# michaelfeil/skyjo_rl

Hardware: AMD Instinct MI355X
Metric: env-steps/sec (whole node) at 65 536 parallel 3-player games (higher is better)
Workload: dtype int8

## Files before the change

### skyjo_rl_amd/csrc/skyjo_step.h

```cpp
#pragma once
#ifndef SKYJO_DEVICE_PARTS
#error "include skyjo_device.h"
#endif

__device__ __forceinline__ void sk_publish_deals(const SkParams &P, int g) {
  const size_t G = (size_t)P.tiles * SK_TILE;
  const int b = P.busy[g];
  if (b) {
    const uint32_t tag = P.plan_tag[g];
    const uint32_t f = __hip_atomic_load(&P.done_flag[g], __ATOMIC_RELAXED, __HIP_MEMORY_SCOPE_AGENT);
    if ((f & 0x7fffffffu) == tag) {
      SK_FENCE_ACQUIRE(P);
      if (!P.cancel[g] && f == tag) P.spare_ready[(size_t)(b - 1) * G + g] = 1;
      P.busy[g] = 0, P.cancel[g] = 0;
    }
  }
}
__device__ __forceinline__ void sk_plan_deals(const SkParams &P, int g, int lane) {
  const size_t G = (size_t)P.tiles * SK_TILE;
  bool need = false, empty = false;
  if (g < P.B) {
    const uint8_t busy = P.busy[g];
    const int head = P.bank_head[g] % SK_BANK;
    const uint32_t consumed = P.deals_consumed[g];
    uint8_t ready[SK_BANK];
#pragma unroll
    for (int k = 0; k < SK_BANK; k++) ready[k] = P.spare_ready[(size_t)k * G + g];
    bool open = true;
    int r = 0;
#pragma unroll
    for (int k = 0; k < SK_BANK; k++) {
      uint8_t f = 0;
#pragma unroll
      for (int j = 0; j < SK_BANK; j++) f = (head + k) % SK_BANK == j ? ready[j] : f;
      open = open && f != 0;
      r += open ? 1 : 0;
    }
    need = !busy && r < SK_BANK;
    empty = need && r == 0;
    if (need) {
      P.busy[g] = (uint8_t)(1 + (head + r) % SK_BANK);
      P.cancel[g] = 0;
      P.plan_ep[g] = consumed + (uint32_t)r;
      P.plan_tag[g] = P.plan_new_tag;
    }
  }
  const unsigned long long be = __ballot(empty);
  if (be && lane == 0) atomicAdd(P.bank_empty + (P.be_add & 1u), (uint32_t)__popcll(be));
}

__device__ __forceinline__ void sk_error_to_host(const SkParams &P, int lane) {
  if (lane == 0) {
    const uint32_t e = __hip_atomic_load(P.dev_error, __ATOMIC_RELAXED, __HIP_MEMORY_SCOPE_AGENT);
    if (e) P.health_host[2] = e;
  }
}
__device__ __forceinline__ void sk_export_raw(const SkParams &P, uint8_t *lp, int g, uint8_t *o) {
  for (int c = 0; c < P.L.chunks; c++) ((uint4 *)o)[c] = LQ(c);
  double *d = (double *)(o + P.L.state_bytes);
  for (int p = 0; p < P.L.N; p++) d[p] = P.rewards[(size_t)g * P.L.N + p], d[P.L.N + p] = P.scores[(size_t)g * P.L.N + p];
  uint32_t *m = (uint32_t *)(d + 2 * P.L.N);
  m[0] = P.rng_mode == SKYJO_RNG_MT19937 ? (uint32_t)P.mt_idx[g] : 0u;
  m[1] = P.done[g];
}

__device__ __forceinline__ uint32_t sk_next_tag(uint32_t t) {
  t = (t + 1u) & 0x7fffffffu;
  return t ? t : 1u;
}
template <bool INDIRECT, bool POLICY, int NP, bool PLANAR = false>
__device__ __forceinline__ void step_body(const SkParams &Pin, const int tile, const int lane, uint32_t *lds_raw, const int32_t *actions,
                                          uint8_t *rec_out, int32_t *act_out, int iters, uint64_t policy_seed, uint64_t iter0,
                                          double *end_rew_out, uint8_t *end_out, uint8_t *raw_out, int raw_stride, const int cycle_len = 0,
                                          const bool defer_ok = true) {
  SkParams P = Pin;
  TRACE_DECL;
  if (NP > 0) P.L = sk_make_layout(NP, INDIRECT ? 1 : 0);
  const int g = tile * SK_TILE + lane;
  const uint32_t lds_tile = (uint32_t)(uintptr_t)(__attribute__((address_space(3))) uint32_t *)lds_raw;
  uint8_t *lp = (uint8_t *)lds_raw + lane * 16;
  uint8_t *stg = (uint8_t *)lds_raw + P.L.chunks * 1024;
  uint8_t *fp = stg + lane * 4;
  const int stg_bytes = (INDIRECT || PLANAR) ? 4096 : SK_TILE * (P.L.rec_bytes + 16);
  uint8_t *ap = stg + stg_bytes + lane * 8;
  constexpr bool DEFER = POLICY && NP > 0 && NP < 8;
  constexpr bool REGACC = NP > 0 && NP < 8;
  constexpr int NACC = REGACC ? SK_ACC_KINDS * NP : 1;
  double racc_store[NACC];
#pragma unroll
  for (int k = 0; k < NACC; k++) racc_store[k] = 0.0;
  double *racc = REGACC ? racc_store : nullptr;
  uint8_t *pendp = DEFER && defer_ok ? stg + stg_bytes + (REGACC ? 0 : SK_ACC_KINDS * P.L.N * 512) + lane * 16 : nullptr;
  int pend_fin = -1;
  if (!REGACC)
    for (int k = 0; k < SK_ACC_KINDS * P.L.N; k++) ACC(k) = 0.0;
  STAMP_DECL;
  if (!POLICY) tile_load(P, P.state, tile, lane, lp);
  else dma_record<true>((const uint8_t *)P.state, (uint32_t)((((size_t)tile * P.L.chunks) * SK_TILE + lane) * 16), lds_tile, P.L.chunks);
  if (P.ov_flags & 1u) sk_publish_deals(P, g);
  sk_vm_drain();
  HdrRegs h;
  HDR_LOAD(h);
  STAMP(0);
  const bool valid = ((h.w0 >> 16) & F_VALID) != 0;
  LaneCounters cnt;
  uint32_t r0 = 0, r1 = 0, r2 = 0, r3 = 0;
  const uint64_t gid = P.game_id0 + (uint64_t)g;
  ObsRegs ob;
  if (valid) obs_load(P, lp, (h.w0 >> 8) & 0xff, ob);
  for (int it = 0; it < iters; it++) {
    const uint64_t iter = iter0 + (uint64_t)it;
    if (POLICY && (it == 0 || (iter & 3) == 0)) {
      philox4x32_10((uint32_t)(iter >> 2), (uint32_t)gid, (uint32_t)(gid >> 32), 0x504F4C00u, (uint32_t)policy_seed,
                    (uint32_t)(policy_seed >> 32), r0, r1, r2, r3);
      for (int k = (int)(iter & 3); k > 0; k--) {
        const uint32_t t = r0;
        r0 = r1, r1 = r2, r2 = r3, r3 = t;
      }
    }
    STAMP_T(3);
    const uint32_t word = r0;
    if (POLICY) {
      r0 = r1, r1 = r2, r2 = r3, r3 = word;
    }
    int a = -1;
    if (valid) {
      const bool over = ((h.w0 >> 16) & F_DONE) != 0;
      if (!POLICY) a = actions[g];
      const bool skip = !POLICY && a == SKYJO_ACTION_SKIP;
      const bool acted = !over && !skip;
      SpareRegs sp;
      const bool resetting = over && P.auto_reset && !skip;
      if (resetting) spare_issue(P, lp, lds_tile, tile, lane, g, sp);
      STAMP_T(4);
      if (!over && !skip) {
        const uint32_t v0 = ob.q0, v1 = ob.q1, v2 = ob.q2;
        STAMP_N(2);
        const uint4 row_pre = LQ(sk_pb(P.L, (h.w0 >> 8) & 0xff) >> 4);
        asm volatile("" ::: "memory");
        if (POLICY) a = policy_pick(h.w0 & 0xff, ob, word);
#ifndef SK_STAMPS_FINE
        STAMP_N(3);
#endif
        apply_action<INDIRECT, NP, POLICY>(P, lp, fp, ap, h, v0, v1, v2, a, g, cnt, st, pendp, pend_fin, row_pre, racc);
#ifdef SK_STAMPS_FINE
        STAMP(6);
#else
        STAMP(5);
#endif
      } else if (!skip) {
        a = -1;
        if (P.auto_reset) {
          bool dealt = true;
          if (!spare_commit(P, lp, g, sp)) {
            dealt = deal_inline(P, lp, fp, g, tile, lane, sp.head);
            cnt.waits++;
          }
          HDR_LOAD(h);
          if (SK_OFTEN(dealt)) {
            h.w0 = (h.w0 & 0x00ffffffu) | ((uint32_t)SKYJO_ST_RESET << 24);
            cnt.resets++;
          }
        } else {
          h.w0 = (h.w0 & 0x00ffffffu) | ((uint32_t)SKYJO_ST_NOOP_DONE << 24);
        }
        STAMP(1);
      } else {
        a = -1;
      }
      if (!POLICY && acted && (unsigned)a >= (unsigned)SKYJO_NUM_ACTIONS) a = -2;
      if (!POLICY && end_out) {
        const bool end = acted && ((h.w0 >> 16) & F_DONE) != 0;
        end_out[g] = end ? 1 : 0;
        for (int q = 0; q < P.L.N; q++) end_rew_out[(size_t)g * P.L.N + q] = end ? P.rewards[(size_t)g * P.L.N + q] : 0.0;
      }
      const uint4 rec_a = LQ(1);
      const uint32_t rec_b = LB(32);
      const uint4 rec_row = LQ((sk_pb(P.L, (h.w0 >> 8) & 0xff) + PB_VIS) >> 4);
      asm volatile("" ::: "memory");
      obs_from_row(rec_row, ob);
      if (rec_out) {
        if (INDIRECT) {
          uint4 rr[4];
          emit_record<INDIRECT>(P, lp, h, ob, a, nullptr, rr, &rec_a, rec_b);
          if (PLANAR) {
            typedef uint32_t u32x4_t __attribute__((ext_vector_type(4)));
            uint8_t *blk = rec_out + ((size_t)it * P.tiles + (size_t)tile) * (SK_TILE * 64) + lane * 16;
#pragma unroll
            for (int p = 0; p < 4; p++) __builtin_nontemporal_store((u32x4_t){rr[p].x, rr[p].y, rr[p].z, rr[p].w}, (u32x4_t *)(blk + p * 1024));
          } else {
#pragma unroll
            for (int p = 0; p < 4; p++) *(uint4 *)(stg + lane * 64 + ((p + (lane >> 1)) & 3) * 16) = rr[p];
          }
        } else if (PLANAR) {
          constexpr int PIECES = NP > 0 ? (((19 + 12 * NP + 3) & ~3) + 32 + 15) / 16 : 1;
          uint32_t wbuf[4 * PIECES];
#pragma unroll
          for (int k = 0; k < 4 * PIECES; k++) wbuf[k] = 0u;
          emit_record<INDIRECT>(P, lp, h, ob, a, (uint8_t *)wbuf, nullptr, &rec_a, rec_b);
          typedef uint32_t u32x4_t __attribute__((ext_vector_type(4)));
          uint8_t *blk = rec_out + ((size_t)it * P.tiles + (size_t)tile) * (SK_TILE * 16 * PIECES) + lane * 16;
#pragma unroll
          for (int p = 0; p < PIECES; p++)
            __builtin_nontemporal_store((u32x4_t){wbuf[4 * p], wbuf[4 * p + 1], wbuf[4 * p + 2], wbuf[4 * p + 3]}, (u32x4_t *)(blk + p * 1024));
        } else {
          emit_record<INDIRECT>(P, lp, h, ob, a, stg + lane * sk_stage_stride(P.L.rec_bytes), nullptr, &rec_a, rec_b);
        }
      }
      if (act_out) __builtin_nontemporal_store(a, &act_out[(size_t)it * P.B + g]);
#ifdef SK_STAMPS_FINE
      STAMP(7);
#else
      STAMP(6);
#endif
    }
    if (DEFER && ((it & (SK_SCORE_EVERY - 1)) == SK_SCORE_EVERY - 1 || it == iters - 1)) {
      if (SK_RARE(__any(pend_fin >= 0))) {
        if (pend_fin >= 0) {
          finish_game_fixed<(NP > 0 && NP < 8) ? NP : 1>(P, pendp, 1024, ap, g, pend_fin, racc);
          pend_fin = -1;
        }
      }
    }
    if (!INDIRECT && !PLANAR && rec_out) {
      typedef uint32_t u32x4_t __attribute__((ext_vector_type(4)));
      const int pieces = P.L.rec_bytes >> 4, stride = sk_stage_stride(P.L.rec_bytes);
      uint8_t *blk = rec_out + ((size_t)it * P.B + (size_t)tile * SK_TILE) * (size_t)P.L.rec_bytes;
      const int live = P.B - tile * SK_TILE;
      for (int q0 = lane; q0 < pieces * SK_TILE; q0 += 4 * SK_TILE) {
        uint4 v[4];
#pragma unroll
        for (int j = 0; j < 4; j++) {
          const int q = q0 + j * SK_TILE, r = q / pieces, p = q - r * pieces;
          if (q < pieces * SK_TILE) v[j] = *(const uint4 *)(stg + r * stride + p * 16);
        }
        if (SK_OFTEN(live >= SK_TILE)) {
#pragma unroll
          for (int j = 0; j < 4; j++) {
            const int q = q0 + j * SK_TILE;
            if (q0 - lane + j * SK_TILE < pieces * SK_TILE)
              __builtin_nontemporal_store((u32x4_t){v[j].x, v[j].y, v[j].z, v[j].w}, (u32x4_t *)(blk + (size_t)q * 16));
          }
        } else {
#pragma unroll
          for (int j = 0; j < 4; j++) {
            const int q = q0 + j * SK_TILE, r = q / pieces;
            if (q < pieces * SK_TILE && r < live)
              __builtin_nontemporal_store((u32x4_t){v[j].x, v[j].y, v[j].z, v[j].w}, (u32x4_t *)(blk + (size_t)q * 16));
          }
        }
      }
    }
    if (INDIRECT && !PLANAR && rec_out) {
      typedef uint32_t u32x4_t __attribute__((ext_vector_type(4)));
      uint8_t *blk = rec_out + ((size_t)it * P.B + (size_t)tile * SK_TILE) * 64;
      const int live = P.B - tile * SK_TILE;
      uint4 v[4];
#pragma unroll
      for (int j = 0; j < 4; j++) {
        const int r = 16 * j + (lane >> 2), p = lane & 3;
        v[j] = *(const uint4 *)(stg + r * 64 + ((p + (r >> 1)) & 3) * 16);
      }
      if (SK_OFTEN(live >= SK_TILE)) {
#pragma unroll
        for (int j = 0; j < 4; j++)
          __builtin_nontemporal_store((u32x4_t){v[j].x, v[j].y, v[j].z, v[j].w}, (u32x4_t *)(blk + j * 1024 + lane * 16));
      } else {
#pragma unroll
        for (int j = 0; j < 4; j++)
          if (16 * j + (lane >> 2) < live)
            __builtin_nontemporal_store((u32x4_t){v[j].x, v[j].y, v[j].z, v[j].w}, (u32x4_t *)(blk + j * 1024 + lane * 16));
      }
    }
    STAMP_T(2);
    if (POLICY && cycle_len && it + 1 < iters && (it + 1) % cycle_len == 0) {
      if (P.busy[g]) (void)wait_deal_done(P, g);
      sk_publish_deals(P, g);
      sk_plan_deals(P, g, lane);
      P.plan_new_tag = sk_next_tag(P.plan_new_tag);
      TRACE_WAIT_BEGIN;
      __syncthreads();
      TRACE_WAIT_END;
    }
  }
  HDR_FLUSH(h);
  tile_store_nt(P, P.state, tile, lane, lp);
  if (!POLICY && raw_out && valid) sk_export_raw(P, lp, g, raw_out + (size_t)g * raw_stride);
  if (P.ov_flags & 2u) {
    if (P.ov_flags & 1u) {
      if (P.busy[g]) (void)wait_deal_done(P, g);
      sk_publish_deals(P, g);
    }
    sk_plan_deals(P, g, lane);
  }
  if (!POLICY) {
    sk_error_to_host(P, lane);
    if (P.host_seq) {
      __threadfence_system();
      if (lane == 0) __hip_atomic_store(&P.health_host[3], P.host_seq, __ATOMIC_RELEASE, __HIP_MEMORY_SCOPE_SYSTEM);
    }
  }
  uint32_t v[7] = {cnt.steps, cnt.episodes, cnt.illegal, cnt.resets, cnt.sum_len, cnt.reshuffles, cnt.waits};
#pragma unroll
  for (int k = 0; k < 7; k++)
    for (int off = 32; off > 0; off >>= 1) v[k] += __shfl_down(v[k], off, 64);
  if (lane == 0) {
    unsigned long long *c = P.tile_counters + (size_t)tile * 8;
#pragma unroll
    for (int k = 0; k < 7; k++) c[k] += v[k];
  }
  if (__any(cnt.episodes | cnt.illegal)) {
    double mine = 0.0;
    if (REGACC) {
#pragma unroll
      for (int k = 0; k < NACC; k++) {
        double x = racc_store[k];
        for (int off = 32; off > 0; off >>= 1) x += __shfl_down(x, off, 64);
        x = __shfl(x, 0, 64);
        mine = lane == k ? x : mine;
      }
    } else {
      for (int k = 0; k < SK_ACC_KINDS * P.L.N; k++) {
        double x = ACC(k);
        for (int off = 32; off > 0; off >>= 1) x += __shfl_down(x, off, 64);
        x = __shfl(x, 0, 64);
        mine = lane == k ? x : mine;
      }
    }
    if (lane < SK_ACC_KINDS * P.L.N)
      P.acc_tile[(size_t)tile * SK_ACC_KINDS * SKYJO_MAX_PLAYERS + (lane / P.L.N) * SKYJO_MAX_PLAYERS + lane % P.L.N] += mine;
  }
  STAMP(7);
  STAMP_STORE;
  TRACE_STORE(0, (uint32_t)(iter0 / (uint64_t)(iters > 0 ? iters : 1)), lane, tile);
}

template <bool INDIRECT, bool POLICY, int NP, bool PLANAR = false>
__global__ __launch_bounds__(SK_TILE) void k_step(SkParams Pin, const int32_t *actions, uint8_t *rec_out,
                                                  int32_t *act_out, int iters, uint64_t policy_seed, uint64_t iter0,
                                                  double *end_rew_out, uint8_t *end_out, uint8_t *raw_out, int raw_stride) {
  extern __shared__ uint32_t lds_raw[];
  step_body<INDIRECT, POLICY, NP, PLANAR>(Pin, (int)blockIdx.x, (int)threadIdx.x, lds_raw, actions, rec_out, act_out, iters, policy_seed, iter0,
                                          end_rew_out, end_out, raw_out, raw_stride);
}

template <bool INDIRECT>
__device__ __forceinline__ void sk_emit_to(const SkParams &P, uint8_t *lp, const HdrRegs &h, const ObsRegs &ob, uint8_t *rec_out, int tile, int lane,
                                           int planar) {
  const int g = tile * SK_TILE + lane;
  if (INDIRECT && planar) {
    uint4 rr[4];
    emit_record<INDIRECT>(P, lp, h, ob, -1, nullptr, rr);
    uint4 *o = (uint4 *)(rec_out + (size_t)tile * SK_TILE * P.L.rec_bytes) + lane;
#pragma unroll
    for (int k = 0; k < 4; k++) o[k * SK_TILE] = rr[k];
  } else {
    emit_record<INDIRECT>(P, lp, h, ob, -1, rec_out + (size_t)g * P.L.rec_bytes);
  }
}

template <bool INDIRECT>
__global__ __launch_bounds__(SK_TILE) void k_observe(SkParams P, const int32_t *players, uint8_t *rec_out, int planar) {
  extern __shared__ uint32_t lds_raw[];
  const int tile = blockIdx.x, lane = threadIdx.x, g = tile * SK_TILE + lane;
  uint8_t *lp = (uint8_t *)lds_raw + lane * 16;
  sk_error_to_host(P, lane);
  tile_load(P, P.state, tile, lane, lp);
  if (!(LB(H_FLAGS) & F_VALID)) return;
  HdrRegs h;
  HDR_LOAD(h);
  int q = players ? players[g] : LB(H_PLAYER);
  q = q < 0 ? 0 : (q >= P.L.N ? P.L.N - 1 : q);
  ObsRegs ob;
  obs_load(P, lp, q, ob);
  sk_emit_to<INDIRECT>(P, lp, h, ob, rec_out, tile, lane, planar);
}

template <bool INDIRECT>
__global__ __launch_bounds__(SK_TILE) void k_reset(SkParams P, const uint8_t *mask, uint8_t *rec_out, uint8_t *raw_out, int raw_stride, int planar) {
  extern __shared__ uint32_t lds_raw[];
  const int tile = blockIdx.x, lane = threadIdx.x, g = tile * SK_TILE + lane;
  uint8_t *lp = (uint8_t *)lds_raw + lane * 16;
  uint8_t *fp = (uint8_t *)lds_raw + P.L.chunks * 1024 + lane * 4;
  if (g >= P.B) return;
  const bool want = !mask || mask[g];
  bool want_counted = false;
  tile_load(P, P.state, tile, lane, lp);
  if (want) {
    const int head = P.bank_head[g] % SK_BANK;
    bool dealt = true;
    if (!consume_spare(P, lp, tile, lane, g, head)) dealt = deal_inline(P, lp, fp, g, tile, lane, head);
    if (dealt) LB(H_STATUS) = SKYJO_ST_RESET;
    want_counted = dealt;
  }
  HdrRegs h;
  HDR_LOAD(h);
  if (rec_out) {
    ObsRegs ob;
    obs_load(P, lp, LB(H_PLAYER), ob);
    sk_emit_to<INDIRECT>(P, lp, h, ob, rec_out, tile, lane, planar);
  }
  if (want) tile_store(P, P.state, tile, lane, lp);
  if (raw_out && (LB(H_FLAGS) & F_VALID)) sk_export_raw(P, lp, g, raw_out + (size_t)g * raw_stride);
  sk_error_to_host(P, lane);
  const unsigned long long wb = __ballot(want_counted);
  if (want_counted && lane == __ffsll((long long)wb) - 1) P.tile_counters[(size_t)tile * 8 + 3] += __popcll(wb);
}
```

### skyjo_rl_amd/csrc/skyjo_transition.h

```cpp
#pragma once
#ifndef SKYJO_DEVICE_PARTS
#error "include skyjo_device.h"
#endif

__device__ __forceinline__ void refresh_minima(const SkParams &P, uint8_t *lp) {
  int ms = LSH(sk_pb(P.L, 0) + PB_SUM), mh = LB(sk_pb(P.L, 0) + PB_HIDDEN);
  for (int q = 1; q < P.L.N; q++) {
    int s = LSH(sk_pb(P.L, q) + PB_SUM), h = LB(sk_pb(P.L, q) + PB_HIDDEN);
    ms = s < ms ? s : ms, mh = h < mh ? h : mh;
  }
  LB(H_MINSUM) = (uint8_t)(int8_t)(ms < 127 ? ms : 127);
  LB(H_MINHID) = (uint8_t)mh;
}

template <class Rng>
__device__ __forceinline__ void reshuffle_discard(const SkParams &P, uint8_t *lp, Rng &r) {
  const int n = LB(H_NDISC), role = LB(H_ROLE), pb = P.L.off_pile;
  const int reg = role ? 0 : 1;
  for (int i = n - 1; i >= 1; i--) {
    int j = (int)rng_interval(r, (uint32_t)i);
    int ai = pb + pile_addr(reg, i), aj = pb + pile_addr(reg, j);
    uint8_t t = LB(ai);
    LB(ai) = LB(aj), LB(aj) = t;
  }
  for (int k = 0; k < n - 1; k++) LB(H_HIST + 2 + LI(pb + pile_addr(reg, k)))--;
  int last = LI(pb + pile_addr(reg, n - 1));
  LB(pb + pile_addr(reg ^ 1, 0)) = (uint8_t)last;
  LB(H_NDRAW) = (uint8_t)(n - 1), LB(H_NDISC) = 1, LB(H_ROLE) = (uint8_t)(role ^ 1);
  LB(H_TOP) = (uint8_t)last;
  int rs = LB(H_RESH);
  LB(H_RESH) = (uint8_t)(rs < 255 ? rs + 1 : 255);
}

#define SK_WAIT_OK 0
#define SK_WAIT_GAVE_UP 1
#define SK_WAIT_TIMEOUT 2
__device__ __forceinline__ int wait_deal_done(const SkParams &P, int g) {
  uint32_t f = 0;
  const uint32_t tag = P.plan_tag[g];
  for (int spin = 0; spin < (1 << P.spin_log2); spin++) {
    f = __hip_atomic_load(&P.done_flag[g], __ATOMIC_RELAXED, __HIP_MEMORY_SCOPE_AGENT);
    if ((f & 0x7fffffffu) == tag) break;
    __builtin_amdgcn_s_sleep(32);
  }
  if ((f & 0x7fffffffu) != tag) {
    atomicOr(P.dev_error, SK_ERR_DEAL_TIMEOUT);
    return SK_WAIT_TIMEOUT;
  }
  SK_FENCE_ACQUIRE(P);
  return (f >> 31) != 0 ? SK_WAIT_GAVE_UP : SK_WAIT_OK;
}

__device__ __forceinline__ uint32_t mt_untwist_y(const uint32_t *mt, int i) {
  uint32_t t = mt[i] ^ mt[i + 397 >= 624 ? i + 397 - 624 : i + 397];
  const uint32_t odd = t >> 31;
  t ^= odd ? 0x9908b0dfu : 0u;
  return (t << 1) | odd;
}
__device__ __forceinline__ void mt_untwist(uint32_t *mt, int from, int to) {
  for (int i = to; i != from;) {
    const int nx = i == 624 ? 0 : i;
    i = nx == 0 ? 623 : nx - 1;
    const uint32_t y = mt_untwist_y(mt, i);
    const int ip1 = i == 623 ? 0 : i + 1;
    mt[ip1] = (mt[ip1] & 0x80000000u) | (y & 0x7fffffffu);
    mt[i] = y & 0x80000000u;
  }
}

__device__ __forceinline__ int mt_rollback(const SkParams &P, uint32_t *mt, int g, int slot, int packed) {
  const size_t G = (size_t)P.tiles * SK_TILE;
  const int snap = P.mt_idx[(size_t)(1 + slot) * G + g];
  int from = (snap & 0xffff) + (snap >> 16), to = (packed & 0xffff) + (packed >> 16);
  from = from >= 624 ? from - 624 : from, to = to >= 624 ? to - 624 : to;
  mt_untwist(mt, from, to);
  return snap;
}

__device__ __forceinline__ void reshuffle_dispatch(const SkParams &P, uint8_t *lp, uint8_t *fp, int g) {
  if (P.rng_mode == SKYJO_RNG_MT19937) {
    const size_t G = (size_t)P.tiles * SK_TILE;
    uint32_t *mt = P.mt + (size_t)g * 624;
    const int head = LB(H_BANK) % SK_BANK;
    const int busy = P.busy[g];
    const bool inflight = busy && !P.cancel[g];
    bool undo_inflight = false;
    if (inflight) {
      const int w = wait_deal_done(P, g);
      if (w == SK_WAIT_TIMEOUT) {
        LB(H_FLAGS) |= F_DONE, LB(H_STATUS) = SKYJO_ST_ERROR, LB(H_NDRAW) = 1;
        P.done[g] = 1;
        for (int q = 0; q < P.L.N; q++) P.rewards[(size_t)g * P.L.N + q] = 0.0;
        return;
      }
      undo_inflight = w == SK_WAIT_OK;
      P.cancel[g] = 1;
    }
    int packed = P.mt_idx[g];
    if (undo_inflight) packed = mt_rollback(P, mt, g, busy - 1, packed);
    for (int k = SK_BANK - 1; k >= 0; k--) {
      const int slot = (head + k) % SK_BANK;
      if (P.spare_ready[(size_t)slot * G + g]) {
        packed = mt_rollback(P, mt, g, slot, packed);
        P.spare_ready[(size_t)slot * G + g] = 0;
      }
    }
    MtStream<16> r;
    r.open(mt, packed, fp);
    reshuffle_discard(P, lp, r);
    P.mt_idx[g] = r.close();
  } else {
    PhiloxStream r;
    r.open(P.seeds[g] + 1, *(uint32_t *)(lp + LIDX(H_EPISODE)), LB(H_RESH), 1u);
    reshuffle_discard(P, lp, r);
  }
}

#define ACC(k) (*(double *)(ap + ((k) << 9)))
__device__ __forceinline__ void acc_add(uint8_t *ap, int k, double v) {
  __hip_atomic_fetch_add(&ACC(k), v, __ATOMIC_RELAXED, __HIP_MEMORY_SCOPE_WAVEFRONT);
}
__device__ __forceinline__ void acc_episode(uint8_t *ap, int N, int p, double score, double reward, int refunded) {
  acc_add(ap, p, score), acc_add(ap, N + p, reward), acc_add(ap, 2 * N + p, reward * reward);
  if (refunded) acc_add(ap, 3 * N + p, (double)refunded);
}

__device__ __forceinline__ void finish_game(const SkParams &P, uint8_t *lp, uint8_t *fp, uint8_t *ap, int g,
                                            int finisher) {
  const int N = P.L.N;
  double *sc = P.scores + (size_t)g * N, *rw = P.rewards + (size_t)g * N;
  int mn = 0, fs = 0;
  for (int p = 0; p < N; p++) {
    int s = 0;
    for (int c = 0; c < 4; c++) {
      int b = sk_pb(P.L, p) + PB_CARDS + 3 * c;
      int t0 = LI(b), t1 = LI(b + 1), t2 = LI(b + 2);
      if (!(t0 == t1 && t1 == t2)) s += t0 + t1 + t2;
    }
    MT_FIFO(p) = (uint32_t)s;
    mn = (p == 0 || s < mn) ? s : mn;
    fs = p == finisher ? s : fs;
  }
  const bool penal = mn != fs;
#define SCORE(p) ((penal && (p) == finisher) ? (double)(int)MT_FIFO(p) * P.score_penalty : (double)(int)MT_FIFO(p))
  double sum;
  if (N < 8) {
    sum = 0.0;
    for (int p = 0; p < N; p++) sum += SCORE(p);
  } else {
    sum = ((SCORE(0) + SCORE(1)) + (SCORE(2) + SCORE(3))) + ((SCORE(4) + SCORE(5)) + (SCORE(6) + SCORE(7)));
    for (int p = 8; p < N; p++) sum += SCORE(p);
  }
  const double mean = sum / (double)N;
  for (int p = 0; p < N; p++) {
    const double d = SCORE(p);
    double r = (-d + mean) + P.mean_reward;
    const int rf = LB(sk_pb(P.L, p) + PB_REFUNDED);
    if (P.reward_refunded != 0.0) r += (double)rf * P.reward_refunded;
    sc[p] = d, rw[p] = r;
    acc_episode(ap, N, p, d, r, rf);
  }
#undef SCORE
  P.done[g] = 1;
}

template <int NP>
__device__ __forceinline__ void finish_game_fixed(const SkParams &P, const uint8_t *rows, int stride, uint8_t *ap, int g, int finisher,
                                                  double *racc = nullptr) {
  double *sc = P.scores + (size_t)g * NP, *rw = P.rewards + (size_t)g * NP;
  int s[NP], refunded[NP];
  int mn = 0, fs = 0;
#pragma unroll
  for (int p = 0; p < NP; p++) {
    const uint4 row = *(const uint4 *)(rows + p * stride);
    const uint32_t c0 = row.x, c1 = row.y, c2 = row.z;
    refunded[p] = (int)(row.w >> 24);
    const uint32_t tri[4] = {c0 & 0xffffffu, (c0 >> 24) | ((c1 & 0xffffu) << 8), (c1 >> 16) | ((c2 & 0xffu) << 16), c2 >> 8};
    int t = 0;
#pragma unroll
    for (int c = 0; c < 4; c++) {
      const int t0 = (int)(int8_t)tri[c], t1 = (int)(int8_t)(tri[c] >> 8), t2 = (int)(int8_t)(tri[c] >> 16);
      t += (t0 == t1 && t1 == t2) ? 0 : t0 + t1 + t2;
    }
    s[p] = t;
    mn = (p == 0 || t < mn) ? t : mn;
    fs = p == finisher ? t : fs;
  }
  const bool penal = mn != fs;
  double d[NP], sum = 0.0;
#pragma unroll
  for (int p = 0; p < NP; p++) {
    d[p] = (penal && p == finisher) ? (double)s[p] * P.score_penalty : (double)s[p];
    sum += d[p];
  }
  const double mean = sum / (double)NP;
#pragma unroll
  for (int p = 0; p < NP; p++) {
    double r = (-d[p] + mean) + P.mean_reward;
    if (P.reward_refunded != 0.0) r += (double)refunded[p] * P.reward_refunded;
    sc[p] = d[p], rw[p] = r;
    if (racc) {
      racc[p] += d[p], racc[NP + p] += r, racc[2 * NP + p] += r * r, racc[3 * NP + p] += (double)refunded[p];
    } else {
      acc_episode(ap, NP, p, d[p], r, refunded[p]);
    }
  }
}

struct HdrRegs {
  uint32_t w0, w1, w2;
};
#define HDR_LOAD(h) ((h).w0 = LW(0), (h).w1 = LW(1), (h).w2 = LW(2))
#define HDR_FLUSH(h) (LW(0) = (h).w0, LW(1) = (h).w1, LW(2) = (h).w2)

__device__ __forceinline__ int byte3(uint32_t a, uint32_t b, uint32_t c, int k) {
  const uint32_t w = k < 4 ? a : (k < 8 ? b : c);
  return (int)(int8_t)(w >> ((k & 3) * 8));
}
__device__ __forceinline__ void put3(uint32_t &a, uint32_t &b, uint32_t &c, int k, int val) {
  const uint32_t sh = (uint32_t)(k & 3) * 8u, m = ~(0xffu << sh), v = ((uint32_t)val & 0xffu) << sh;
  if (k < 4) a = (a & m) | v;
  else if (k < 8) b = (b & m) | v;
  else c = (c & m) | v;
}
__device__ __forceinline__ void hist_add(uint8_t *lp, int value, int delta) {
  const int b = H_HIST + 2 + value;
  uint32_t *w = (uint32_t *)(lp + LIDX(b & ~3));
  const uint32_t d = (uint32_t)delta << ((b & 3) * 8);
  __hip_atomic_fetch_add(w, d, __ATOMIC_RELAXED, __HIP_MEMORY_SCOPE_WAVEFRONT);
}
__device__ __forceinline__ uint32_t swar_nonzero01(uint32_t x) {
  return ((((x & 0x7f7f7f7fu) + 0x7f7f7f7fu) | x) & 0x80808080u) >> 7;
}
__device__ __forceinline__ uint32_t pack12(uint32_t a, uint32_t b, uint32_t c) {
  return ((a * 0x00204081u >> 21) & 0xfu) | (((b * 0x00204081u >> 21) & 0xfu) << 4) |
         (((c * 0x00204081u >> 21) & 0xfu) << 8);
}

struct ObsRegs {
  uint32_t q0, q1, q2, nz0, nz1, nz2, hd0, hd1, hd2;
};
__device__ __forceinline__ void obs_from_row(const uint4 &row, ObsRegs &o) {
  o.q0 = row.x, o.q1 = row.y, o.q2 = row.z;
  o.nz0 = swar_nonzero01(o.q0 ^ 0xf2f2f2f2u);
  o.nz1 = swar_nonzero01(o.q1 ^ 0xf2f2f2f2u);
  o.nz2 = swar_nonzero01(o.q2 ^ 0xf2f2f2f2u);
  o.hd0 = swar_nonzero01(o.q0 ^ 0x0f0f0f0fu) ^ 0x01010101u;
  o.hd1 = swar_nonzero01(o.q1 ^ 0x0f0f0f0fu) ^ 0x01010101u;
  o.hd2 = swar_nonzero01(o.q2 ^ 0x0f0f0f0fu) ^ 0x01010101u;
}
__device__ __forceinline__ void obs_load(const SkParams &P, uint8_t *lp, int q, ObsRegs &o) {
  const uint4 row = LQ((sk_pb(P.L, q) + PB_VIS) >> 4);
  obs_from_row(row, o);
}

__device__ __forceinline__ int policy_pick(int phase, const ObsRegs &o, uint32_t word) {
  if (phase == 0) return 24 + (int)__umulhi(word, 2u);
  uint32_t legal = pack12(o.nz0, o.nz1, o.nz2) | (pack12(o.hd0, o.hd1, o.hd2) << 12);
  const int n = __popc(legal);
  if (n == 0) return 24;
  int k = (int)__umulhi(word, (uint32_t)n), pos = 0;
  int c = __popc(legal & 0xfffu);
  if (k >= c) k -= c, pos = 12, legal >>= 12;
  c = __popc(legal & 0x3fu);
  if (k >= c) k -= c, pos += 6, legal >>= 6;
  c = __popc(legal & 0x7u);
  if (k >= c) k -= c, pos += 3, legal >>= 3;
  c = (int)(legal & 1u);
  if (k >= c) {
    k -= c, pos += 1;
    c = (int)((legal >> 1) & 1u);
    if (k >= c) pos += 1;
  }
  return pos;
}

template <bool INDIRECT, int NP, bool TRUSTED>
__device__ __forceinline__ void apply_action(const SkParams &P, uint8_t *lp, uint8_t *fp, uint8_t *ap, HdrRegs &h, uint32_t v0,
                                             uint32_t v1, uint32_t v2, int a, int g, LaneCounters &cnt, Stamps &st,
                                             uint8_t *pendp, int &pend_fin, const uint4 &row_pre, double *racc = nullptr) {
  const int N = P.L.N;
  const int phase = h.w0 & 0xff, p = (h.w0 >> 8) & 0xff;
  const int blk = sk_pb(P.L, p), cardb = blk + PB_CARDS, visb = blk + PB_VIS, pb = P.L.off_pile;
  const unsigned ua = (unsigned)a;
  int slot = 0, sv = 0;
  bool legal;
  if (ua < 24u) {
    slot = a < 12 ? a : a - 12;
    sv = byte3(v0, v1, v2, slot);
    legal = phase == 1 && (TRUSTED || (a < 12 ? sv != SKYJO_REFUNDED : sv == SKYJO_HAND_NONE));
  } else {
    legal = (TRUSTED || ua <= 25u) && phase == 0;
  }
  if (!legal) {
    double *rw = P.rewards + (size_t)g * N;
    for (int q = 0; q < N; q++) rw[q] = q == p ? P.illegal_reward : 0.0;
    if (NP > 0 && racc) {
#pragma unroll
      for (int q = 0; q < (NP > 0 ? NP : 1); q++)
        racc[NP + q] += q == p ? P.illegal_reward : 0.0, racc[2 * NP + q] += q == p ? P.illegal_reward * P.illegal_reward : 0.0;
    } else {
      acc_add(ap, N + p, P.illegal_reward), acc_add(ap, 2 * N + p, P.illegal_reward * P.illegal_reward);
    }
    h.w0 = (h.w0 & 0x0000ffffu) | ((((h.w0 >> 16) & 0xffu) | F_DONE) << 16) | ((uint32_t)SKYJO_ST_ILLEGAL << 24);
    P.done[g] = 1;
    cnt.illegal++;
    return;
  }
  const int eplen = (int)(h.w2 & 0xffffu) + 1;
  h.w2 = (h.w2 & 0xffff0000u) | (uint32_t)eplen;
  h.w0 &= 0x00ffffffu;
  cnt.steps++;
  if (phase == 0) {
    const int role = (h.w1 >> 16) & 1;
    int nd = h.w1 & 0xff;
    const int ns = (h.w1 >> 8) & 0xff;
    const int hidden_p = (int)((row_pre.w >> 16) & 0xffu);
    int pile_top = LI(pb + pile_addr(role, nd > 0 ? nd - 1 : 0));
    const int disc_top = LI(pb + pile_addr(role ^ 1, ns > 0 ? ns - 1 : 0));
    const int disc_below = LI(pb + pile_addr(role ^ 1, ns > 1 ? ns - 2 : 0));

    if (hidden_p == 0) {
      h.w0 |= (uint32_t)(F_TERMINATED | F_DONE) << 16;
      LB(H_FINISHER) = (uint8_t)p;
      if (NP > 0 && NP < 8) {
        constexpr int NQ = (NP > 0 && NP < 8) ? NP : 1;
        P.done[g] = 1;
        if (pendp) {
#pragma unroll
          for (int q = 0; q < NQ; q++) *(uint4 *)(pendp + q * 1024) = LQ(sk_pb(P.L, q) >> 4);
          pend_fin = p;
        } else {
          finish_game_fixed<NQ>(P, lp + (P.L.off_players >> 4) * 1024, 2048, ap, g, p, racc);
        }
      } else {
        finish_game(P, lp, fp, ap, g, p);
      }
      cnt.episodes++;
      cnt.sum_len += eplen;
#ifdef SK_STAMPS_FINE
      STAMP(3);
#endif
      return;
    }
    const bool from_pile = a == 24;
    if (from_pile && nd == 0) {
      HDR_FLUSH(h);
      reshuffle_dispatch(P, lp, fp, g);
      HDR_LOAD(h);
      cnt.reshuffles++;
      nd = h.w1 & 0xff;
      pile_top = LI(pb + pile_addr((h.w1 >> 16) & 1, nd - 1));
    }
    int hand;
    if (from_pile) {
      hand = pile_top;
      h.w1 = (h.w1 & 0xffffff00u) | (uint32_t)(nd - 1);
    } else {
      hand = disc_top;
      hist_add(lp, hand, -1);
      const int top = ns > 1 ? disc_below : -3;
      h.w1 = (h.w1 & 0x00ff00ffu) | ((uint32_t)(ns - 1) << 8) | (((uint32_t)top & 0xffu) << 24);
    }
    h.w2 = (h.w2 & 0x00ffffffu) | (((uint32_t)hand & 0xffu) << 24);
    h.w0 = (h.w0 & 0xffffff00u) | 1u;
#ifdef SK_STAMPS_FINE
    STAMP(3);
#endif
    return;
  }
  STAMP_N(4);
  const int hand = (int)(int8_t)(h.w2 >> 24);
  const int reg = ((h.w1 >> 16) & 1) ^ 1;
  int ns = (h.w1 >> 8) & 0xff;
  const uint4 row = row_pre;
  const uint32_t c0 = row.x, c1 = row.y, c2 = row.z;
  int sum = (int)(int16_t)(row.w & 0xffffu), hid = (int)((row.w >> 16) & 0xffu), refunded = (int)(row.w >> 24);
  int oms = 1 << 20, omh = 1 << 20;
  for (int q = 0; q < N; q++) {
    const uint32_t cq = LW((sk_pb(P.L, q) + PB_SUM) >> 2);
    const int s = (int)(int16_t)(cq & 0xffffu), hq = (int)((cq >> 16) & 0xffu);
    oms = (q != p && s < oms) ? s : oms, omh = (q != p && hq < omh) ? hq : omh;
  }
#ifdef SK_STAMPS_FINE
  STAMP(5);
#endif
  const bool swap = a < 12, was_hidden = sv == SKYJO_HAND_NONE;
  const int under = byte3(c0, c1, c2, slot);
  const int shown = swap ? hand : under, gone = swap ? under : hand;
  LB(pb + pile_addr(reg, ns)) = (uint8_t)gone;
  ns++;
  hist_add(lp, gone, 1);
  LB(cardb + slot) = (uint8_t)shown;
  LB(visb + slot) = (uint8_t)shown;
  put3(v0, v1, v2, slot, shown);
  sum += shown - (was_hidden ? 0 : under);
  hid -= was_hidden ? 1 : 0;
  if (!INDIRECT) {
    if (!was_hidden) hist_add(lp, under, -1);
    hist_add(lp, shown, 1);
  }
  int top = gone;
  {
    const uint32_t tri[4] = {v0 & 0xffffffu, (v0 >> 24) | ((v1 & 0xffffu) << 8), (v1 >> 16) | ((v2 & 0xffu) << 16), v2 >> 8};
    bool full[4];
#pragma unroll
    for (int c = 0; c < 4; c++) {
      const uint32_t b0 = tri[c] & 0xffu;
      full[c] = ((tri[c] ^ (tri[c] >> 8)) & 0xffffu) == 0 && b0 != (uint32_t)SKYJO_HAND_NONE && b0 != ((uint32_t)SKYJO_REFUNDED & 0xffu);
    }
    if (full[0] | full[1] | full[2] | full[3]) {
#pragma unroll
      for (int c = 0; c < 4; c++)
        if (full[c]) {
          const int t0 = (int)(int8_t)(tri[c] & 0xff);
          for (int k = 0; k < 3; k++) {
            LB(cardb + 3 * c + k) = (uint8_t)(int8_t)SKYJO_REFUNDED;
            LB(visb + 3 * c + k) = (uint8_t)(int8_t)SKYJO_REFUNDED;
            LB(pb + pile_addr(reg, ns)) = 0;
            ns++;
          }
          hist_add(lp, 0, 3);
          if (!INDIRECT) hist_add(lp, t0, -3);
          sum -= 3 * t0;
          top = 0;
        }
      refunded++;
    }
  }
  LW((blk + PB_SUM) >> 2) = ((uint32_t)sum & 0xffffu) | ((uint32_t)hid << 16) | ((uint32_t)refunded << 24);
  __hip_atomic_fetch_add((uint32_t *)(lp + LIDX(blk + PB_PLACED)), 1u, __ATOMIC_RELAXED, __HIP_MEMORY_SCOPE_WAVEFRONT);
  const int ms = sum < oms ? sum : oms, mh = hid < omh ? hid : omh;
  LB(H_MINSUM) = (uint8_t)(int8_t)(ms < 127 ? ms : 127);
  LB(H_MINHID) = (uint8_t)mh;
  h.w1 = (h.w1 & 0x00ff00ffu) | ((uint32_t)ns << 8) | (((uint32_t)top & 0xffu) << 24);
  h.w2 = (h.w2 & 0x00ffffffu) | ((uint32_t)SKYJO_HAND_NONE << 24);
  const int np = p + 1 == N ? 0 : p + 1;
  h.w0 = (h.w0 & 0xffff0000u) | ((uint32_t)np << 8);
}
```

Before: 49.07 billion.

## Specialize policy step by wave-uniform phase with dedicated draw-turn path

Under the built-in policy, a wave ballot checks whether every valid lane is in the draw phase, every lane is in the place phase, or the lanes are mixed. It then runs a phase-specialized instance of the turn body, so uniform waves avoid divergent execution of both phase branches. A dedicated draw_turn function patches the record header in registers instead of reloading it from LDS. The place-phase path preloads the other players' sum words before apply_action. Compile-time flags replace runtime null checks on the register accumulator. The cost is code-size growth from three instantiations, with possible register pressure and instruction-cache effects.

Result: slower. 46.39 billion (-5.5%).

```diff
diff --git a/skyjo_rl_amd/csrc/skyjo_step.h b/skyjo_rl_amd/csrc/skyjo_step.h
--- a/skyjo_rl_amd/csrc/skyjo_step.h
+++ b/skyjo_rl_amd/csrc/skyjo_step.h
@@ -68,6 +68,10 @@
   t = (t + 1u) & 0x7fffffffu;
   return t ? t : 1u;
 }
+template <int V>
+struct SkPhase {
+  static constexpr int value = V;
+};
 template <bool INDIRECT, bool POLICY, int NP, bool PLANAR = false>
 __device__ __forceinline__ void step_body(const SkParams &Pin, const int tile, const int lane, uint32_t *lds_raw, const int32_t *actions,
                                           uint8_t *rec_out, int32_t *act_out, int iters, uint64_t policy_seed, uint64_t iter0,
@@ -108,6 +112,7 @@
   const uint64_t gid = P.game_id0 + (uint64_t)g;
   ObsRegs ob;
   if (valid) obs_load(P, lp, (h.w0 >> 8) & 0xff, ob);
+  const unsigned long long valid_mask = __ballot(valid);
   for (int it = 0; it < iters; it++) {
     const uint64_t iter = iter0 + (uint64_t)it;
     if (POLICY && (it == 0 || (iter & 3) == 0)) {
@@ -124,100 +129,126 @@
       r0 = r1, r1 = r2, r2 = r3, r3 = word;
     }
     int a = -1;
-    if (valid) {
-      const bool over = ((h.w0 >> 16) & F_DONE) != 0;
-      if (!POLICY) a = actions[g];
-      const bool skip = !POLICY && a == SKYJO_ACTION_SKIP;
-      const bool acted = !over && !skip;
-      SpareRegs sp;
-      const bool resetting = over && P.auto_reset && !skip;
-      if (resetting) spare_issue(P, lp, lds_tile, tile, lane, g, sp);
-      STAMP_T(4);
-      if (!over && !skip) {
-        const uint32_t v0 = ob.q0, v1 = ob.q1, v2 = ob.q2;
-        STAMP_N(2);
-        const uint4 row_pre = LQ(sk_pb(P.L, (h.w0 >> 8) & 0xff) >> 4);
-        asm volatile("" ::: "memory");
-        if (POLICY) a = policy_pick(h.w0 & 0xff, ob, word);
+    auto turn = [&](auto mode) __attribute__((always_inline)) {
+      constexpr int PH = decltype(mode)::value;
+      if (valid) {
+        const bool over = PH != 0 && ((h.w0 >> 16) & F_DONE) != 0;
+        if (!POLICY) a = actions[g];
+        const bool skip = !POLICY && a == SKYJO_ACTION_SKIP;
+        const bool acted = !over && !skip;
+        SpareRegs sp;
+        const bool resetting = over && P.auto_reset && !skip;
+        if (resetting) spare_issue(P, lp, lds_tile, tile, lane, g, sp);
+        STAMP_T(4);
+        uint4 rec_a;
+        uint32_t rec_b;
+        if (PH == 0) {
+          a = 24 + (int)__umulhi(word, 2u);
+          draw_turn<NP>(P, lp, fp, ap, h, a, g, cnt, pendp, pend_fin, racc, rec_a, rec_b);
+          STAMP(5);
+        } else if (!over && !skip) {
+          const uint32_t v0 = ob.q0, v1 = ob.q1, v2 = ob.q2;
+          STAMP_N(2);
+          const uint4 row_pre = LQ(sk_pb(P.L, (h.w0 >> 8) & 0xff) >> 4);
+          constexpr int NMIN = (PH == 1 && NP > 0) ? NP : 1;
+          uint32_t minw[NMIN];
+          if (PH == 1 && NP > 0) {
+#pragma unroll
+            for (int q = 0; q < NMIN; q++) minw[q] = LW((sk_pb(P.L, q) + PB_SUM) >> 2);
+          }
+          asm volatile("" ::: "memory");
+          if (POLICY) a = policy_pick(PH == 1 ? 1 : (int)(h.w0 & 0xff), ob, word);
 #ifndef SK_STAMPS_FINE
-        STAMP_N(3);
+          STAMP_N(3);
 #endif
-        apply_action<INDIRECT, NP, POLICY>(P, lp, fp, ap, h, v0, v1, v2, a, g, cnt, st, pendp, pend_fin, row_pre, racc);
+          apply_action<INDIRECT, NP, POLICY, PH>(P, lp, fp, ap, h, v0, v1, v2, a, g, cnt, st, pendp, pend_fin, row_pre, racc,
+                                                 (PH == 1 && NP > 0) ? minw : nullptr);
 #ifdef SK_STAMPS_FINE
+          STAMP(6);
+#else
+          STAMP(5);
+#endif
+        } else if (!skip) {
+          a = -1;
+          if (P.auto_reset) {
+            bool dealt = true;
+            if (!spare_commit(P, lp, g, sp)) {
+              dealt = deal_inline(P, lp, fp, g, tile, lane, sp.head);
+              cnt.waits++;
+            }
+            HDR_LOAD(h);
+            if (SK_OFTEN(dealt)) {
+              h.w0 = (h.w0 & 0x00ffffffu) | ((uint32_t)SKYJO_ST_RESET << 24);
+              cnt.resets++;
+            }
+          } else {
+            h.w0 = (h.w0 & 0x00ffffffu) | ((uint32_t)SKYJO_ST_NOOP_DONE << 24);
+          }
+          STAMP(1);
+        } else {
+          a = -1;
+        }
+        if (!POLICY && acted && (unsigned)a >= (unsigned)SKYJO_NUM_ACTIONS) a = -2;
+        if (!POLICY && end_out) {
+          const bool end = acted && ((h.w0 >> 16) & F_DONE) != 0;
+          end_out[g] = end ? 1 : 0;
+          for (int q = 0; q < P.L.N; q++) end_rew_out[(size_t)g * P.L.N + q] = end ? P.rewards[(size_t)g * P.L.N + q] : 0.0;
+        }
+        if (PH != 0) {
+          rec_a = LQ(1);
+          rec_b = LB(32);
+          const uint4 rec_row = LQ((sk_pb(P.L, (h.w0 >> 8) & 0xff) + PB_VIS) >> 4);
+          asm volatile("" ::: "memory");
+          obs_from_row(rec_row, ob);
+        }
+        if (rec_out) {
+          if (INDIRECT) {
+            uint4 rr[4];
+            emit_record<INDIRECT>(P, lp, h, ob, a, nullptr, rr, &rec_a, rec_b);
+            if (PLANAR) {
+              typedef uint32_t u32x4_t __attribute__((ext_vector_type(4)));
+              uint8_t *blk = rec_out + ((size_t)it * P.tiles + (size_t)tile) * (SK_TILE * 64) + lane * 16;
+#pragma unroll
+              for (int p = 0; p < 4; p++) __builtin_nontemporal_store((u32x4_t){rr[p].x, rr[p].y, rr[p].z, rr[p].w}, (u32x4_t *)(blk + p * 1024));
+            } else {
+#pragma unroll
+              for (int p = 0; p < 4; p++) *(uint4 *)(stg + lane * 64 + ((p + (lane >> 1)) & 3) * 16) = rr[p];
+            }
+          } else if (PLANAR) {
+            constexpr int PIECES = NP > 0 ? (((19 + 12 * NP + 3) & ~3) + 32 + 15) / 16 : 1;
+            uint32_t wbuf[4 * PIECES];
+#pragma unroll
+            for (int k = 0; k < 4 * PIECES; k++) wbuf[k] = 0u;
+            emit_record<INDIRECT>(P, lp, h, ob, a, (uint8_t *)wbuf, nullptr, &rec_a, rec_b);
+            typedef uint32_t u32x4_t __attribute__((ext_vector_type(4)));
+            uint8_t *blk = rec_out + ((size_t)it * P.tiles + (size_t)tile) * (SK_TILE * 16 * PIECES) + lane * 16;
+#pragma unroll
+            for (int p = 0; p < PIECES; p++)
+              __builtin_nontemporal_store((u32x4_t){wbuf[4 * p], wbuf[4 * p + 1], wbuf[4 * p + 2], wbuf[4 * p + 3]}, (u32x4_t *)(blk + p * 1024));
+          } else {
+            emit_record<INDIRECT>(P, lp, h, ob, a, stg + lane * sk_stage_stride(P.L.rec_bytes), nullptr, &rec_a, rec_b);
+          }
+        }
+        if (act_out) __builtin_nontemporal_store(a, &act_out[(size_t)it * P.B + g]);
+#ifdef SK_STAMPS_FINE
+        STAMP(7);
+#else
         STAMP(6);
-#else
-        STAMP(5);
 #endif
-      } else if (!skip) {
-        a = -1;
-        if (P.auto_reset) {
-          bool dealt = true;
-          if (!spare_commit(P, lp, g, sp)) {
-            dealt = deal_inline(P, lp, fp, g, tile, lane, sp.head);
-            cnt.waits++;
-          }
-          HDR_LOAD(h);
-          if (SK_OFTEN(dealt)) {
-            h.w0 = (h.w0 & 0x00ffffffu) | ((uint32_t)SKYJO_ST_RESET << 24);
-            cnt.resets++;
-          }
-        } else {
-          h.w0 = (h.w0 & 0x00ffffffu) | ((uint32_t)SKYJO_ST_NOOP_DONE << 24);
-        }
-        STAMP(1);
-      } else {
-        a = -1;
-      }
-      if (!POLICY && acted && (unsigned)a >= (unsigned)SKYJO_NUM_ACTIONS) a = -2;
-      if (!POLICY && end_out) {
-        const bool end = acted && ((h.w0 >> 16) & F_DONE) != 0;
-        end_out[g] = end ? 1 : 0;
-        for (int q = 0; q < P.L.N; q++) end_rew_out[(size_t)g * P.L.N + q] = end ? P.rewards[(size_t)g * P.L.N + q] : 0.0;
-      }
-      const uint4 rec_a = LQ(1);
-      const uint32_t rec_b = LB(32);
-      const uint4 rec_row = LQ((sk_pb(P.L, (h.w0 >> 8) & 0xff) + PB_VIS) >> 4);
-      asm volatile("" ::: "memory");
-      obs_from_row(rec_row, ob);
-      if (rec_out) {
-        if (INDIRECT) {
-          uint4 rr[4];
-          emit_record<INDIRECT>(P, lp, h, ob, a, nullptr, rr, &rec_a, rec_b);
-          if (PLANAR) {
-            typedef uint32_t u32x4_t __attribute__((ext_vector_type(4)));
-            uint8_t *blk = rec_out + ((size_t)it * P.tiles + (size_t)tile) * (SK_TILE * 64) + lane * 16;
-#pragma unroll
-            for (int p = 0; p < 4; p++) __builtin_nontemporal_store((u32x4_t){rr[p].x, rr[p].y, rr[p].z, rr[p].w}, (u32x4_t *)(blk + p * 1024));
-          } else {
-#pragma unroll
-            for (int p = 0; p < 4; p++) *(uint4 *)(stg + lane * 64 + ((p + (lane >> 1)) & 3) * 16) = rr[p];
-          }
-        } else if (PLANAR) {
-          constexpr int PIECES = NP > 0 ? (((19 + 12 * NP + 3) & ~3) + 32 + 15) / 16 : 1;
-          uint32_t wbuf[4 * PIECES];
-#pragma unroll
-          for (int k = 0; k < 4 * PIECES; k++) wbuf[k] = 0u;
-          emit_record<INDIRECT>(P, lp, h, ob, a, (uint8_t *)wbuf, nullptr, &rec_a, rec_b);
-          typedef uint32_t u32x4_t __attribute__((ext_vector_type(4)));
-          uint8_t *blk = rec_out + ((size_t)it * P.tiles + (size_t)tile) * (SK_TILE * 16 * PIECES) + lane * 16;
-#pragma unroll
-          for (int p = 0; p < PIECES; p++)
-            __builtin_nontemporal_store((u32x4_t){wbuf[4 * p], wbuf[4 * p + 1], wbuf[4 * p + 2], wbuf[4 * p + 3]}, (u32x4_t *)(blk + p * 1024));
-        } else {
-          emit_record<INDIRECT>(P, lp, h, ob, a, stg + lane * sk_stage_stride(P.L.rec_bytes), nullptr, &rec_a, rec_b);
-        }
-      }
-      if (act_out) __builtin_nontemporal_store(a, &act_out[(size_t)it * P.B + g]);
-#ifdef SK_STAMPS_FINE
-      STAMP(7);
-#else
-      STAMP(6);
-#endif
+      }
+    };
+    if (POLICY) {
+      const unsigned long long not_draw = __ballot(valid && (h.w0 & (((uint32_t)F_DONE << 16) | 0xffu)) != 0);
+      if (not_draw == 0) turn(SkPhase<0>());
+      else if (not_draw == valid_mask) turn(SkPhase<1>());
+      else turn(SkPhase<-1>());
+    } else {
+      turn(SkPhase<-1>());
     }
     if (DEFER && ((it & (SK_SCORE_EVERY - 1)) == SK_SCORE_EVERY - 1 || it == iters - 1)) {
       if (SK_RARE(__any(pend_fin >= 0))) {
         if (pend_fin >= 0) {
-          finish_game_fixed<(NP > 0 && NP < 8) ? NP : 1>(P, pendp, 1024, ap, g, pend_fin, racc);
+          finish_game_fixed<(NP > 0 && NP < 8) ? NP : 1, REGACC>(P, pendp, 1024, ap, g, pend_fin, racc);
           pend_fin = -1;
         }
       }
diff --git a/skyjo_rl_amd/csrc/skyjo_transition.h b/skyjo_rl_amd/csrc/skyjo_transition.h
--- a/skyjo_rl_amd/csrc/skyjo_transition.h
+++ b/skyjo_rl_amd/csrc/skyjo_transition.h
@@ -164,7 +164,7 @@
   P.done[g] = 1;
 }
 
-template <int NP>
+template <int NP, bool REGS = false>
 __device__ __forceinline__ void finish_game_fixed(const SkParams &P, const uint8_t *rows, int stride, uint8_t *ap, int g, int finisher,
                                                   double *racc = nullptr) {
   double *sc = P.scores + (size_t)g * NP, *rw = P.rewards + (size_t)g * NP;
@@ -199,7 +199,7 @@
     double r = (-d[p] + mean) + P.mean_reward;
     if (P.reward_refunded != 0.0) r += (double)refunded[p] * P.reward_refunded;
     sc[p] = d[p], rw[p] = r;
-    if (racc) {
+    if (REGS) {
       racc[p] += d[p], racc[NP + p] += r, racc[2 * NP + p] += r * r, racc[3 * NP + p] += (double)refunded[p];
     } else {
       acc_episode(ap, NP, p, d[p], r, refunded[p]);
@@ -275,12 +275,13 @@
   return pos;
 }
 
-template <bool INDIRECT, int NP, bool TRUSTED>
+template <bool INDIRECT, int NP, bool TRUSTED, int PH = -1>
 __device__ __forceinline__ void apply_action(const SkParams &P, uint8_t *lp, uint8_t *fp, uint8_t *ap, HdrRegs &h, uint32_t v0,
                                              uint32_t v1, uint32_t v2, int a, int g, LaneCounters &cnt, Stamps &st,
-                                             uint8_t *pendp, int &pend_fin, const uint4 &row_pre, double *racc = nullptr) {
+                                             uint8_t *pendp, int &pend_fin, const uint4 &row_pre, double *racc = nullptr,
+                                             const uint32_t *minw = nullptr) {
   const int N = P.L.N;
-  const int phase = h.w0 & 0xff, p = (h.w0 >> 8) & 0xff;
+  const int phase = PH < 0 ? (int)(h.w0 & 0xff) : PH, p = (h.w0 >> 8) & 0xff;
   const int blk = sk_pb(P.L, p), cardb = blk + PB_CARDS, visb = blk + PB_VIS, pb = P.L.off_pile;
   const unsigned ua = (unsigned)a;
   int slot = 0, sv = 0;
@@ -295,7 +296,7 @@
   if (!legal) {
     double *rw = P.rewards + (size_t)g * N;
     for (int q = 0; q < N; q++) rw[q] = q == p ? P.illegal_reward : 0.0;
-    if (NP > 0 && racc) {
+    if (NP > 0 && NP < 8) {
 #pragma unroll
       for (int q = 0; q < (NP > 0 ? NP : 1); q++)
         racc[NP + q] += q == p ? P.illegal_reward : 0.0, racc[2 * NP + q] += q == p ? P.illegal_reward * P.illegal_reward : 0.0;
@@ -331,7 +332,7 @@
           for (int q = 0; q < NQ; q++) *(uint4 *)(pendp + q * 1024) = LQ(sk_pb(P.L, q) >> 4);
           pend_fin = p;
         } else {
-          finish_game_fixed<NQ>(P, lp + (P.L.off_players >> 4) * 1024, 2048, ap, g, p, racc);
+          finish_game_fixed<NQ, true>(P, lp + (P.L.off_players >> 4) * 1024, 2048, ap, g, p, racc);
         }
       } else {
         finish_game(P, lp, fp, ap, g, p);
@@ -377,10 +378,18 @@
   const uint32_t c0 = row.x, c1 = row.y, c2 = row.z;
   int sum = (int)(int16_t)(row.w & 0xffffu), hid = (int)((row.w >> 16) & 0xffu), refunded = (int)(row.w >> 24);
   int oms = 1 << 20, omh = 1 << 20;
-  for (int q = 0; q < N; q++) {
-    const uint32_t cq = LW((sk_pb(P.L, q) + PB_SUM) >> 2);
-    const int s = (int)(int16_t)(cq & 0xffffu), hq = (int)((cq >> 16) & 0xffu);
-    oms = (q != p && s < oms) ? s : oms, omh = (q != p && hq < omh) ? hq : omh;
+  if (PH == 1 && NP > 0) {
+#pragma unroll
+    for (int q = 0; q < (NP > 0 ? NP : 1); q++) {
+      const int s = (int)(int16_t)(minw[q] & 0xffffu), hq = (int)((minw[q] >> 16) & 0xffu);
+      oms = (q != p && s < oms) ? s : oms, omh = (q != p && hq < omh) ? hq : omh;
+    }
+  } else {
+    for (int q = 0; q < N; q++) {
+      const uint32_t cq = LW((sk_pb(P.L, q) + PB_SUM) >> 2);
+      const int s = (int)(int16_t)(cq & 0xffffu), hq = (int)((cq >> 16) & 0xffu);
+      oms = (q != p && s < oms) ? s : oms, omh = (q != p && hq < omh) ? hq : omh;
+    }
   }
 #ifdef SK_STAMPS_FINE
   STAMP(5);
@@ -438,3 +447,69 @@
   const int np = p + 1 == N ? 0 : p + 1;
   h.w0 = (h.w0 & 0xffff0000u) | ((uint32_t)np << 8);
 }
+
+template <int NP>
+__device__ __forceinline__ void draw_turn(const SkParams &P, uint8_t *lp, uint8_t *fp, uint8_t *ap, HdrRegs &h, int a, int g,
+                                          LaneCounters &cnt, uint8_t *pendp, int &pend_fin, double *racc, uint4 &rec_a, uint32_t &rec_b) {
+  const int p = (h.w0 >> 8) & 0xff, pb = P.L.off_pile;
+  const int role = (h.w1 >> 16) & 1;
+  int nd = h.w1 & 0xff;
+  const int ns = (h.w1 >> 8) & 0xff;
+  const uint32_t cw = LW((sk_pb(P.L, p) + PB_SUM) >> 2);
+  int pile_top = LI(pb + pile_addr(role, nd > 0 ? nd - 1 : 0));
+  const int disc_top = LI(pb + pile_addr(role ^ 1, ns > 0 ? ns - 1 : 0));
+  const int disc_below = LI(pb + pile_addr(role ^ 1, ns > 1 ? ns - 2 : 0));
+  rec_a = LQ(1);
+  rec_b = LB(32);
+  asm volatile("" ::: "memory");
+  const int eplen = (int)(h.w2 & 0xffffu) + 1;
+  h.w2 = (h.w2 & 0xffff0000u) | (uint32_t)eplen;
+  h.w0 &= 0x00ffffffu;
+  cnt.steps++;
+  if (((cw >> 16) & 0xffu) == 0) {
+    h.w0 |= (uint32_t)(F_TERMINATED | F_DONE) << 16;
+    LB(H_FINISHER) = (uint8_t)p;
+    if (NP > 0 && NP < 8) {
+      constexpr int NQ = (NP > 0 && NP < 8) ? NP : 1;
+      P.done[g] = 1;
+      if (pendp) {
+#pragma unroll
+        for (int q = 0; q < NQ; q++) *(uint4 *)(pendp + q * 1024) = LQ(sk_pb(P.L, q) >> 4);
+        pend_fin = p;
+      } else {
+        finish_game_fixed<NQ, true>(P, lp + (P.L.off_players >> 4) * 1024, 2048, ap, g, p, racc);
+      }
+    } else {
+      finish_game(P, lp, fp, ap, g, p);
+    }
+    cnt.episodes++;
+    cnt.sum_len += eplen;
+    return;
+  }
+  const bool from_pile = a == 24;
+  if (from_pile && nd == 0) {
+    HDR_FLUSH(h);
+    reshuffle_dispatch(P, lp, fp, g);
+    HDR_LOAD(h);
+    cnt.reshuffles++;
+    nd = h.w1 & 0xff;
+    pile_top = LI(pb + pile_addr((h.w1 >> 16) & 1, nd - 1));
+    rec_a = LQ(1);
+    rec_b = LB(32);
+  }
+  int hand;
+  if (from_pile) {
+    hand = pile_top;
+    h.w1 = (h.w1 & 0xffffff00u) | (uint32_t)(nd - 1);
+  } else {
+    hand = disc_top;
+    hist_add(lp, hand, -1);
+    const uint32_t k = (uint32_t)(H_HIST + 2 - 16 + hand), w = k >> 2, d = 1u << ((k & 3u) * 8u);
+    rec_a.x -= w == 0 ? d : 0u, rec_a.y -= w == 1 ? d : 0u, rec_a.z -= w == 2 ? d : 0u, rec_a.w -= w == 3 ? d : 0u;
+    rec_b -= w == 4 ? d : 0u;
+    const int top = ns > 1 ? disc_below : -3;
+    h.w1 = (h.w1 & 0x00ff00ffu) | ((uint32_t)(ns - 1) << 8) | (((uint32_t)top & 0xffu) << 24);
+  }
+  h.w2 = (h.w2 & 0x00ffffffu) | (((uint32_t)hand & 0xffu) << 24);
+  h.w0 = (h.w0 & 0xffffff00u) | 1u;
+}
```
